# pxl-th/Trace.jl

Hardware: AMD Instinct MI355X
Metric: Mray/s (all bounces) (higher is better)
Workload: dtype f32

## Files before the change

### trace.jl_amd/csrc/th_kernels.h

```cpp
#pragma once
#include "th_device.h"

namespace th {

constexpr int kBlock = 256;
constexpr int kStackLds = 32;
constexpr int kStackSpill = 32;

struct PathQueue {
    float4* o;
    float4* d;
    float4* beta;
};
struct ShadowQueue {
    float4* o;
    float4* d;
    float4* c;
};
constexpr int kMaxDepth = 62;
constexpr int kSeg = 32;
constexpr uint32_t kSegGran = 256;
#ifndef TH_CTR_STRIDE
#define TH_CTR_STRIDE 32
#endif
// ... 111 lines not shown
#else
    return p;
#endif
}
TH_D size_t film_index(uint32_t layout, uint32_t npix, uint32_t spp, uint32_t s, uint32_t pix) {
    return layout ? ((size_t)(pix >> 6) * spp + s) * 64u + film_chunk_pos(pix & 63u) : (size_t)s * npix + pix;
}
struct MapSpp {
    const uint32_t* counts;
    uint32_t max_spp;
};
TH_D uint32_t spp_of_frame(uint32_t spp) { return spp; }
TH_D uint32_t spp_of_frame(const MapSpp& m) { return m.max_spp; }
TH_D uint32_t spp_of_pixel(uint32_t spp, uint32_t) { return spp; }
TH_D uint32_t spp_of_pixel(const MapSpp& m, uint32_t pix) { return m.counts[pix]; }
constexpr uint32_t kFilmPackSide = 0x80000000u;
constexpr uint32_t kFilmPackOverflow = 0xffffffffu;
constexpr uint32_t kFilmPackException = 0xffffffffu;
struct FilmSideTable {
    uint4* desc;
    uint32_t* count;
    uint32_t cap;
};
TH_D uint32_t film_pack_word(const FilmSideTable& side, uint4 d, int px, int py);
TH_D uint4 film_splat_desc(const DeviceSensor& se, int px, int py, uint64_t key) {
    const float rx = se.filter_radius[0], ry = se.filter_radius[1];
    const float inv_rx = 1.0f / rx, inv_ry = 1.0f / ry;
    const float pfx = (float)px + ts_uniform(key, TS_DIM_FILM_X), pfy = (float)py + ts_uniform(key, TS_DIM_FILM_Y);
    const float dpx = pfx - 0.5f, dpy = pfy - 0.5f;
    const float p0x = __builtin_ceilf(dpx - rx), p0y = __builtin_ceilf(dpy - ry);
    const float p1x = __builtin_floorf(dpx + rx) + 1.0f, p1y = __builtin_floorf(dpy + ry) + 1.0f;
    const int nx = (int)(p1x - p0x) + 1, ny = (int)(p1y - p0y) + 1;
    uint32_t oxw = 0, oyw = 0;
    for (int c = 0; c < 8; ++c) {
        const float X = p0x + (float)c, Y = p0y + (float)c;
        oxw |= (uint32_t)((int)jclamp(__builtin_ceilf(fabs_((X - dpx) * inv_rx * 16.0f)), 1.0f, 16.0f) - 1) << (4 * c);
        oyw |= (uint32_t)((int)jclamp(__builtin_floorf(fabs_((Y - dpy) * inv_ry * 16.0f)), 1.0f, 16.0f) - 1) << (4 * c);
    }
    return make_uint4(((uint32_t)(int)p0x & 0xffffu) | ((uint32_t)(int)p0y << 16), (uint32_t)nx | ((uint32_t)ny << 8), oxw, oyw);
}
TH_D uint32_t film_pack_desc(uint4 d, int px, int py) {
    const int p0x = (int)(short)(d.x & 0xffffu), p0y = (int)(short)(d.x >> 16);
    const uint32_t nx = d.y & 0xffu, ny = (d.y >> 8) & 0xffu;
    const int ox = px - p0x, oy = py - p0y;
    if (ox < 0 || ox > 1 || oy < 0 || oy > 1 || nx < 1u || nx > 3u || ny < 1u || ny > 3u) return kFilmPackException;
    return (uint32_t)ox | ((uint32_t)oy << 1) | ((nx - 1u) << 2) | ((ny - 1u) << 4) | ((d.z & 0xfffu) << 6) | ((d.w & 0xfffu) << 18);
}
TH_D uint32_t film_pack_word(const FilmSideTable& side, uint4 d, int px, int py) {
    const uint32_t w = film_pack_desc(d, px, py);
    if (w != kFilmPackException) return w;
    const uint32_t j = atomicAdd(side.count, 1u);
    if (j >= side.cap || j >= 0x7fffffffu) return kFilmPackOverflow;
    side.desc[j] = d;
    return kFilmPackSide | j;
}

TH_D void generate_ray(const DeviceSensor& se, f2 film, f2 lens, float time_u, f3& o, f3& d, float& time) {
    const f3 p_camera = xf_point(se.raster_to_camera, mk3(film.x, film.y, 0.0f));
    o = splat3(0.0f);
    d = normalize(p_camera);
    if (se.lens_radius > 0.0f) {
        const f2 pl = concentric_sample_disk(lens);
        const f2 p_lens{se.lens_radius * pl.x, se.lens_radius * pl.y};
        const float t = se.focal_distance / d.z;
        const f3 p_focus = o + d * t;
        o = mk3(p_lens.x, p_lens.y, 0.0f);
        d = normalize(p_focus - o);
    }
    time = (1 - time_u) * se.shutter_open + time_u * se.shutter_close;
    o = xf_point(se.camera_to_world, o);
    d = xf_vec(se.camera_to_world, d);
    d = normalize(d);
}

struct MapJobs {
    const uint32_t* jobs;
    uint32_t job0;
};
TH_D uint32_t raygen_slot(uint32_t slot0, uint32_t i) { return slot0 + i; }
TH_D uint32_t raygen_slot(const MapJobs& m, uint32_t i) { return m.jobs[m.job0 + i]; }
template <int TH_ONE_COPY = 0, class SLOT0 = uint32_t> __global__ __launch_bounds__(kBlock) void k_raygen(const DeviceSensor* __restrict__ sep, SLOT0 slot0, uint32_t n, uint64_t seed, uint32_t sample_offset,
                                                   PathQueue q, uint32_t cap, Counters* ctr, float4* __restrict__ Lf = nullptr, uint32_t spp_frame = 0, FilmSideTable side = FilmSideTable{nullptr, nullptr, 0}) {
    const DeviceSensor& se = *sep;
    for (uint32_t i = blockIdx.x * kBlock + threadIdx.x; i < n; i += gridDim.x * kBlock) {
        uint32_t slot = raygen_slot(slot0, i);
        const SlotInfo si = slot_info(se, slot);
        const uint64_t key = ts_stream_key(seed, si.px, si.py, sample_offset + si.sample);
        if (Lf) {
            slot = (uint32_t)film_index(1u, (uint32_t)(se.sb_w * se.band_rows), spp_frame, si.sample, si.pix);
            Lf[slot] = make_float4(0.0f, 0.0f, 0.0f, __uint_as_float(film_pack_word(side, film_splat_desc(se, si.px, si.py, key), si.px, si.py)));
        }
        const f2 film{(float)si.px + ts_uniform(key, TS_DIM_FILM_X), (float)si.py + ts_uniform(key, TS_DIM_FILM_Y)};
        const f2 lens{ts_uniform(key, TS_DIM_LENS_X), ts_uniform(key, TS_DIM_LENS_Y)};
        f3 o, d;
        float time;
        generate_ray(se, film, lens, ts_uniform(key, TS_DIM_TIME), o, d, time);
        d = check_direction(d);
        const uint32_t w = i >> 6;
        const uint32_t phys = (w % kSeg) * cap + (w / kSeg) * 64u + (i & 63u);
        q.o[phys] = make_float4(o.x, o.y, o.z, __uint_as_float(slot));
        q.d[phys] = make_float4(d.x, d.y, d.z, __uint_as_float((uint32_t)key));
        q.beta[phys] = make_float4(1.0f, 1.0f, 1.0f, __uint_as_float((uint32_t)(key >> 32)));
    }
    if (blockIdx.x == 0 && threadIdx.x < kSeg) {
        const uint32_t sgm = threadIdx.x, W = (n + 63u) >> 6;
        uint32_t cnt = ((W + kSeg - 1 - sgm) / kSeg) * 64u;
        if (W > 0 && (W - 1) % kSeg == sgm && (n & 63u)) cnt -= 64u - (n & 63u);
        ctr->n_queue[0][sgm * kCtrStride] = cnt;
    }
}

template <int TH_ONE_COPY = 0> __global__ __launch_bounds__(kBlock) void k_apply_poison(float4* __restrict__ L, const uint8_t* __restrict__ poison, uint64_t n) {
    for (uint64_t i = (uint64_t)blockIdx.x * kBlock + threadIdx.x; i < n; i += (uint64_t)gridDim.x * kBlock) {
        const uint32_t p = poison[i];
        if (p) {
            float4 l = L[i];
            const float nanv = __builtin_nanf("");
            if (p & 1u) l.x += nanv;
            if (p & 2u) l.y += nanv;
            if (p & 4u) l.z += nanv;
            L[i] = l;
        }
    }
}

struct Hit {
    float t;
    int prim;
    float b1, b2;
};
TH_D bool slab_test(float4 n0, float4 n1, f3 o, f3 inv_d, bool negx, bool negy, bool negz, float t_max) {
    float tx_min = ((negx ? n1.x : n0.x) - o.x) * inv_d.x;
    float tx_max = ((negx ? n0.x : n1.x) - o.x) * inv_d.x;
    const float ty_min = ((negy ? n1.y : n0.y) - o.y) * inv_d.y;
    const float ty_max = ((negy ? n0.y : n1.y) - o.y) * inv_d.y;
    if (tx_min > ty_max || ty_min > tx_max) return false;
    if (ty_min > tx_min) tx_min = ty_min;
    if (ty_max > tx_max) tx_max = ty_max;
    const float tz_min = ((negz ? n1.z : n0.z) - o.z) * inv_d.z;
    const float tz_max = ((negz ? n0.z : n1.z) - o.z) * inv_d.z;
    if (tx_min > tz_max || tz_min > tx_max) return false;
    if (tz_min > tx_min) tx_min = tz_min;
    if (tz_max < tx_max) tx_max = tz_max;
    return tx_min < t_max && tx_max > 0.0f;
}

template <bool ANY, bool COUNT>
TH_D bool traverse(const DeviceScene& sc, f3 o, f3 d, float t_max, uint32_t (*stk)[kBlock], Hit* hit, uint32_t& n_nodes, uint32_t& n_prims) {
    const f3 inv_d = mk3(1.0f / d.x, 1.0f / d.y, 1.0f / d.z);
    const bool negx = d.x < 0.0f, negy = d.y < 0.0f, negz = d.z < 0.0f;
    uint32_t spill[kStackSpill];
    int sp = 0;
    uint32_t cur = 0;
    bool found = false;
    if (sc.n_nodes == 0) return false;
    const uint32_t tid = threadIdx.x;
    while (true) {
        const float4 n0 = sc.nodes[2 * cur], n1 = sc.nodes[2 * cur + 1];
        if (COUNT) n_nodes++;
        bool pop = true;
        if (slab_test(n0, n1, o, inv_d, negx, negy, negz, t_max)) {
            const uint32_t a = __float_as_uint(n0.w), flags = __float_as_uint(n1.w);
            if ((flags & 3u) == 3u) {
                const uint32_t cnt = flags >> 2;
                for (uint32_t k = 0; k < cnt; ++k) {
                    const uint32_t slot = a + k;
                    const float4 p0 = sc.prims[3 * slot];
                    const uint32_t meta = __float_as_uint(p0.w);
                    if (COUNT) n_prims++;
                    if (meta & PRIM_SPHERE) {
                        SphereHit sh;
                        if (sphere_intersect<false>(sc.spheres[__float_as_uint(p0.x)], o, d, t_max, sh)) {
                            if (ANY) return true;
                            t_max = sh.t;
                            found = true;
                            hit->prim = (int)slot;
                            hit->b1 = hit->b2 = 0.0f;
                        }
                    } else {
                        const float4 p1 = sc.prims[3 * slot + 1], p2 = sc.prims[3 * slot + 2];
                        TriTest tt;
                        if (tri_intersect<!ANY>(mk3(p0.x, p0.y, p0.z), mk3(p1.x, p1.y, p1.z), mk3(p2.x, p2.y, p2.z), o, d, t_max, &tt)) {
                            if (ANY) return true;
                            t_max = tt.t;
                            found = true;
                            hit->prim = (int)slot;
                            hit->b1 = tt.bary.x;
                            hit->b2 = tt.bary.y;
                        }
                    }
                }
            } else {
                const uint32_t axis = flags & 3u;
                const bool neg = axis == 0 ? negx : (axis == 1 ? negy : negz);
                const uint32_t far_child = neg ? cur + 1 : a;
                cur = neg ? a : cur + 1;
                if (sp < kStackLds)
                    stk[sp][tid] = far_child;
                else if (sp < kStackLds + kStackSpill)
                    spill[sp - kStackLds] = far_child;
                sp++;
                pop = false;
            }
        }
        if (pop) {
            if (sp == 0) break;
            sp--;
            cur = sp < kStackLds ? stk[sp][tid] : (sp < kStackLds + kStackSpill ? spill[sp - kStackLds] : 0u);
        }
    }
    if (!ANY) hit->t = t_max;
    return found;
}

template <bool COUNT>
__global__ __launch_bounds__(kBlock) void k_trace_closest(DeviceScene sc, SegQueue q, const float4* __restrict__ ro, const float4* __restrict__ rd, const float* __restrict__ tmax_or_null,
                                                          float4* __restrict__ hits, Counters* ctr) {
    __shared__ uint32_t stk[kStackLds][kBlock];
    __shared__ SegView sv;
    seg_load(q, sv);
    const uint32_t total = sv.prefix[kSeg];
    uint32_t nn = 0, np = 0;
    uint32_t seg = 0;
    for (uint32_t flat = blockIdx.x * kBlock + threadIdx.x; flat < total; flat += gridDim.x * kBlock) {
        uint32_t lb;
        seg_locate_from(sv, flat & ~63u, seg, lb);
        const uint32_t local = lb + (flat & 63u);
        if (local >= sv.count[seg]) continue;
        const uint32_t i = seg_phys(q, seg, local);
        const float4 o4 = ro[i], d4 = rd[i];
        Hit h;
        h.prim = -1;
        h.b1 = h.b2 = 0.0f;
        const float t0 = tmax_or_null ? tmax_or_null[i] : kInf;
        const bool found = traverse<false, COUNT>(sc, mk3(o4.x, o4.y, o4.z), mk3(d4.x, d4.y, d4.z), t0, stk, &h, nn, np);
        hits[i] = make_float4(found ? h.t : kInf, __int_as_float(found ? h.prim : -1), h.b1, h.b2);
    }
    if (ctr) {
        if (blockIdx.x == 0 && threadIdx.x == 0) atomicAdd(&ctr->closest_total, (unsigned long long)seg_total(sv));
        if (COUNT) {
            const unsigned long long sn = wave_sum(nn), spr = wave_sum(np);
            if (lane_id() == 0) {
                atomicAdd(&ctr->nodes_closest, sn);
                atomicAdd(&ctr->prims_closest, spr);
            }
        }
    }
}

template <bool COUNT>
__global__ __launch_bounds__(kBlock) void k_trace_any(DeviceScene sc, SegQueue q, const float4* __restrict__ ro, const float4* __restrict__ rd, const float4* __restrict__ contrib,
                                                      const float* __restrict__ tmax_or_null, float4* __restrict__ L, uint8_t* __restrict__ occluded, Counters* ctr) {
    __shared__ uint32_t stk[kStackLds][kBlock];
    __shared__ SegView sv;
    seg_load(q, sv);
    const uint32_t total = sv.prefix[kSeg];
    uint32_t nn = 0, np = 0;
    uint32_t seg = 0;
    for (uint32_t flat = blockIdx.x * kBlock + threadIdx.x; flat < total; flat += gridDim.x * kBlock) {
        uint32_t lb;
        seg_locate_from(sv, flat & ~63u, seg, lb);
        const uint32_t local = lb + (flat & 63u);
        if (local >= sv.count[seg]) continue;
        const uint32_t i = seg_phys(q, seg, local);
        const float4 o4 = ro[i], d4 = rd[i];
        const float t0 = tmax_or_null ? tmax_or_null[i] : kInf;
        const bool occ = traverse<true, COUNT>(sc, mk3(o4.x, o4.y, o4.z), mk3(d4.x, d4.y, d4.z), t0, stk, nullptr, nn, np);
        if (L) {
            const uint32_t slot = __float_as_uint(o4.w);
            if (!occ) {
                const float4 c = contrib[i];
                float4 l = L[slot];
                l.x += c.x;
                l.y += c.y;
                l.z += c.z;
                L[slot] = l;
            } else {
                const uint32_t poison = __float_as_uint(d4.w);
                if (poison) {
                    float4 l = L[slot];
                    const float nanv = __builtin_nanf("");
                    if (poison & 1u) l.x += nanv;
                    if (poison & 2u) l.y += nanv;
                    if (poison & 4u) l.z += nanv;
                    L[slot] = l;
                }
            }
        } else {
            occluded[i] = occ ? 1 : 0;
        }
    }
    if (ctr) {
        if (blockIdx.x == 0 && threadIdx.x == 0) atomicAdd(&ctr->shadow_total, (unsigned long long)seg_total(sv));
        if (COUNT) {
            const unsigned long long sn = wave_sum(nn), spr = wave_sum(np);
            if (lane_id() == 0) {
                atomicAdd(&ctr->nodes_shadow, sn);
                atomicAdd(&ctr->prims_shadow, spr);
            }
        }
    }
}

template <bool TRI_ONLY = false, bool TAN = true>
TH_D bool rebuild_shading(const DeviceScene& sc, int prim, f3 o, f3 d, Shading& sh, uint32_t& material, const float4* bary = nullptr, f3* fast_r = nullptr) {
    const float4* rec = sc.shade + 8 * (size_t)prim;
    const float4 p0 = rec[0], p1 = rec[1], p2 = rec[2];
    const float4 na = rec[3], nb = rec[4], nc = rec[5];
    const float4 cn = rec[6], cs = rec[7];
    const uint32_t meta = __float_as_uint(p0.w);
    material = meta & PRIM_MATERIAL_MASK;
    if (fast_r) *fast_r = mk3(na.w, nb.w, nc.w);
    if (!TRI_ONLY && (meta & PRIM_SPHERE)) {
        const SphereRec& s = sc.spheres[__float_as_uint(p0.x)];
        SphereHit h;
        if (!sphere_intersect<true>(s, o, d, kInf, h)) return false;
        sh = shade_sphere(s, h, d);
        return true;
    }
    const f3 v0 = mk3(p0.x, p0.y, p0.z), v1 = mk3(p1.x, p1.y, p1.z), v2 = mk3(p2.x, p2.y, p2.z);
    TriTest tt;
    if (bary)
        tt.bary = mk3(bary->z, bary->w, bary->x);
    else if (!tri_intersect<true>(v0, v1, v2, o, d, kInf, &tt))
        return false;
    const bool has_n = (meta & PRIM_HAS_NORMALS) != 0;
    const TriConstants tc{mk3(cn.x, cn.y, cn.z), mk3(cs.x, cs.y, cs.z)};
    const float4* tan = (TAN && sc.tri_tan && (meta & PRIM_HAS_TANGENTS)) ? sc.tri_tan + 3 * (size_t)prim : nullptr;
    sh = shade_triangle(v0, v1, v2, has_n, mk3(na.x, na.y, na.z), mk3(nb.x, nb.y, nb.z), mk3(nc.x, nc.y, nc.z), (meta & PRIM_FLIP) != 0, tt.bary, d, &tc, tan);
    return true;
}
template <int TH_ONE_COPY = 0> __global__ __launch_bounds__(kBlock) void k_shade_constants(float4* __restrict__ shade, const float4* __restrict__ prims, const float4* __restrict__ nrm, const float4* __restrict__ uv, uint32_t n_prims) {
    for (uint32_t k = blockIdx.x * kBlock + threadIdx.x; k < n_prims; k += gridDim.x * kBlock) {
        float4* rec = shade + 8 * (size_t)k;
        const float4 p0 = prims[3 * (size_t)k], p1 = prims[3 * (size_t)k + 1], p2 = prims[3 * (size_t)k + 2];
        rec[0] = p0;
        rec[1] = p1;
        rec[2] = p2;
        for (int j = 0; j < 3; ++j) rec[3 + j] = nrm[3 * (size_t)k + j];
        float4 c6 = make_float4(0.0f, 0.0f, 0.0f, 0.0f), c7 = c6;
        if (!(__float_as_uint(p0.w) & PRIM_SPHERE)) {
            float uvs[6];
            bool has_uv = false;
            if (uv) {
                const float4 a = uv[2 * (size_t)k], b = uv[2 * (size_t)k + 1];
                uvs[0] = a.x, uvs[1] = a.y, uvs[2] = a.z, uvs[3] = a.w, uvs[4] = b.x, uvs[5] = b.y;
                has_uv = b.z != 0.0f;
            }
            const TriConstants tc = triangle_constants(mk3(p0.x, p0.y, p0.z), mk3(p1.x, p1.y, p1.z), mk3(p2.x, p2.y, p2.z), has_uv ? uvs : nullptr);
            c6 = make_float4(tc.n.x, tc.n.y, tc.n.z, 0.0f);
            c7 = make_float4(tc.ss.x, tc.ss.y, tc.ss.z, 0.0f);
        }
        rec[6] = c6;
        rec[7] = c7;
    }
}

#ifndef TH_SHADE_WAVES
#define TH_SHADE_WAVES 4
#endif
struct ShadeStream {
    const uint32_t* tags_in;
    uint32_t* tags_out;
    uint32_t term_stride;
    uint8_t* poison;
};
struct ShadeOut {
    bool want_shadow, want_next;
    float4 so4, sd4, sc4, no4, nd4, nb4;
    uint32_t next_depth;
};
template <bool STREAM, bool FAST, bool TAN = true, bool DIRL = false>
TH_D void shade_vertex(const DeviceScene& sc, const PathQueue& qin, const float4* __restrict__ hits, float4* __restrict__ L, uint32_t i, int depth_fixed, int max_depth,
                       uint32_t hits_have_bary, const ShadeStream& ss, ShadeOut& out) {
    const float4 h4 = hits[i];
    const int prim = __float_as_int(h4.y);
    const float4 o4 = qin.o[i], d4 = qin.d[i], b4 = qin.beta[i];
    const int depth = STREAM ? (int)ss.tags_in[i] : depth_fixed;
    const uint32_t slot = STREAM ? (uint32_t)(depth - 1) * ss.term_stride + __float_as_uint(o4.w) : __float_as_uint(o4.w);
    const f3 o = mk3(o4.x, o4.y, o4.z), d = mk3(d4.x, d4.y, d4.z);
    f3 beta = mk3(b4.x, b4.y, b4.z);
    Shading sh;
    uint32_t material;
    f3 fast_r;
    if (!(rebuild_shading<FAST, TAN>(sc, prim, o, d, sh, material, hits_have_bary ? &h4 : nullptr, &fast_r) && material != PRIM_NO_MATERIAL)) return;
    const LobeSet& bsdf = sc.materials[FAST ? 0u : material].set[1];
    const bool lambert = FAST || bsdf_is_single_lambert(bsdf);
    Lobe lam;
    if (FAST) {
        lam.kind = LOBE_LAMBERT_R;
        lam.type = BSDF_DIFFUSE | BSDF_REFLECTION;
        lam.r[0] = fast_r.x;
        lam.r[1] = fast_r.y;
        lam.r[2] = fast_r.z;
    } else if (lambert) {
        lam = bsdf.lobe[0];
    }
    const uint64_t key = ((uint64_t)__float_as_uint(b4.w) << 32) | (uint64_t)__float_as_uint(d4.w);
    const uint32_t v = (uint32_t)(depth - 1);
    const f3 wo = -d;
    const uint32_t poison = ((isnan_(beta.x) || isinf_(beta.x)) ? 1u : 0u) | ((isnan_(beta.y) || isinf_(beta.y)) ? 2u : 0u) | ((isnan_(beta.z) || isinf_(beta.z)) ? 4u : 0u);
    bool direct_added = false;
    if (sc.n_lights > 0) {
        const int nl = (int)sc.n_lights;
        int ln = (int)__builtin_ceilf(ts_uniform(key, ts_vertex_dim(v, TS_V_LIGHT_PICK)) * (float)nl);
        if (ln > nl) ln = nl;
        if (ln < 1) ln = 1;
        const float light_pdf = 1.0f / (float)nl;
        const LightRec light = nl == 1 ? uniform_load(sc.lights, 0u) : sc.lights[ln - 1];
        const LightSample ls = sample_li<DIRL>(light, sh.p);
        if (ls.pdf > 0.0f && !is_black(ls.radiance)) {
            const f3 f = (lambert ? lambert_bsdf_f(lam, sh, sh.wo, ls.wi) : bsdf_f(bsdf, sh, sh.wo, ls.wi, BSDF_ALL & ~BSDF_SPECULAR)) * fabs_(dot(ls.wi, sh.ns));
            if (!is_black(f)) {
                const f3 fl = f * ls.radiance;
                const f3 Ld1 = splat3(0.0f) + (ls.pdf == 1.0f ? fl : fl / ls.pdf);
                const f3 Ld = light_pdf == 1.0f ? Ld1 : Ld1 / light_pdf;
                const f3 c = beta * Ld;
                const f3 lp = light_target<DIRL>(light, sh.p);
                const f3 dir = lp - sh.p;
                const f3 org = sh.p + 1e-6f * dir;
                const f3 cd = check_direction(dir);
                out.so4 = make_float4(org.x, org.y, org.z, __uint_as_float(slot));
                out.sd4 = make_float4(cd.x, cd.y, cd.z, __uint_as_float(poison));
                out.sc4 = make_float4(c.x, c.y, c.z, 0.0f);
                out.want_shadow = true;
                direct_added = true;
            }
        }
    }
    if (!direct_added && poison && ss.poison) {
        ss.poison[slot] |= (uint8_t)poison;
    } else if (!direct_added && poison) {
        float4 l = L[slot];
        const float nanv = __builtin_nanf("");
        if (poison & 1u) l.x += nanv;
        if (poison & 2u) l.y += nanv;
        if (poison & 4u) l.z += nanv;
        L[slot] = l;
    }
    if (depth < max_depth) {
        const f2 u{ts_uniform(key, ts_vertex_dim(v, TS_V_BSDF_U0)), ts_uniform(key, ts_vertex_dim(v, TS_V_BSDF_U1))};
        const BsdfSample bs = lambert ? lambert_bsdf_sample_f(lam, sh, wo, u) : bsdf_sample_f(bsdf, sh, wo, u, BSDF_ALL);
        if (!(bs.pdf == 0.0f || is_black(bs.f))) {
            beta = beta * (bs.f * fabs_(dot(bs.wi, sh.ns)) / bs.pdf);
            const float by = to_Y(beta);
            bool alive = true;
            if (by < 0.25f) {
                const float cont = jmin(1.0f, by);
                if (ts_uniform(key, ts_vertex_dim(v, TS_V_RR)) > cont)
                    alive = false;
                else
                    beta = beta / cont;
            }
            if (alive) {
                const f3 org = sh.p + 1e-6f * bs.wi;
                const f3 nd = check_direction(bs.wi);
                out.no4 = make_float4(org.x, org.y, org.z, o4.w);
                out.nd4 = make_float4(nd.x, nd.y, nd.z, d4.w);
                out.nb4 = make_float4(beta.x, beta.y, beta.z, b4.w);
                out.next_depth = (uint32_t)(depth + 1);
                out.want_next = true;
            }
        }
    }
}

template <bool STREAM, bool TAN = true, bool DIRL = false>
__global__ __launch_bounds__(kBlock) __attribute__((amdgpu_waves_per_eu(TH_SHADE_WAVES))) void k_shade_path(DeviceScene sc, const DeviceSensor* __restrict__ sep, PathQueue qin, PathQueue qout, ShadowQueue sq, uint32_t cap,
                                                       const float4* __restrict__ hits, float4* __restrict__ L, Counters* ctr, int row, int depth_fixed, int max_depth, uint32_t hits_have_bary,
                                                       ShadeStream ss) {
    __shared__ SegView sv;
    __shared__ uint32_t s_ring[kBlock / 64][128];
    const SegQueue qv{ctr->n_queue[row], cap, 0u};
    seg_load(qv, sv);
    const uint32_t total = sv.prefix[kSeg];
    const uint32_t lane = lane_id(), wv = threadIdx.x >> 6;
    const unsigned long long lt_mask = (1ull << lane) - 1ull;
    const uint32_t seg_out = ((blockIdx.x * kBlock + threadIdx.x) >> 6) % kSeg;
    uint32_t ring_head = 0, ring_cnt = 0;
    auto emit = [&](const ShadeOut& e) {
        uint32_t si, ni;
        wave_compact2(e.want_shadow, &ctr->n_shadow[row][seg_out * kCtrStride], e.want_next, &ctr->n_queue[row + 1][seg_out * kCtrStride], si, ni);
        si += seg_out * cap;
        ni += seg_out * cap;
        if (e.want_shadow) {
            sq.o[si] = e.so4;
            sq.d[si] = e.sd4;
            sq.c[si] = e.sc4;
        }
        if (e.want_next) {
            qout.o[ni] = e.no4;
            qout.d[ni] = e.nd4;
            qout.beta[ni] = e.nb4;
            if (STREAM) ss.tags_out[ni] = e.next_depth;
        }
    };
    uint32_t seg_in = 0;
    for (uint32_t flat = blockIdx.x * kBlock + threadIdx.x; flat < total; flat += gridDim.x * kBlock) {
        uint32_t lb;
        seg_locate_from(sv, flat & ~63u, seg_in, lb);
        const uint32_t local = lb + (flat & 63u);
        const uint32_t i = seg_in * cap + local;
        int cls = 0;
        if (local < sv.count[seg_in]) {
            const int prim = __float_as_int(hits[i].y);
            if (prim >= 0) {
                cls = (__float_as_uint(sc.shade[8 * (size_t)prim].w) & PRIM_FAST) ? 1 : 2;
            }
        }
        ShadeOut e;
        e.want_shadow = e.want_next = false;
        e.next_depth = 0;
        if (cls == 1) shade_vertex<STREAM, true, TAN, DIRL>(sc, qin, hits, L, i, depth_fixed, max_depth, hits_have_bary, ss, e);
        emit(e);
        const unsigned long long m2 = __ballot(cls == 2);
        if (m2) {
            if (cls == 2) s_ring[wv][(ring_head + ring_cnt + (uint32_t)__popcll(m2 & lt_mask)) & 127u] = i;
            ring_cnt += (uint32_t)__popcll(m2);
            __builtin_amdgcn_fence(__ATOMIC_ACQ_REL, "wavefront");
            if (ring_cnt >= 64u) {
                const uint32_t j = s_ring[wv][(ring_head + lane) & 127u];
                ShadeOut g;
                g.want_shadow = g.want_next = false;
                g.next_depth = 0;
                shade_vertex<STREAM, false, TAN, DIRL>(sc, qin, hits, L, j, depth_fixed, max_depth, hits_have_bary, ss, g);
                emit(g);
                ring_head = (ring_head + 64u) & 127u;
                ring_cnt -= 64u;
                __builtin_amdgcn_fence(__ATOMIC_ACQ_REL, "wavefront");
            }
        }
    }
    if (ring_cnt) {
        ShadeOut g;
        g.want_shadow = g.want_next = false;
        g.next_depth = 0;
        if (lane < ring_cnt) shade_vertex<STREAM, false, TAN, DIRL>(sc, qin, hits, L, s_ring[wv][(ring_head + lane) & 127u], depth_fixed, max_depth, hits_have_bary, ss, g);
        emit(g);
    }
}
template <int TH_ONE_COPY = 0> __global__ __launch_bounds__(kBlock) void k_fold_terms(const float4* __restrict__ terms, uint64_t n_slots, uint32_t n_depths, float4* __restrict__ L) {
    for (uint64_t i = (uint64_t)blockIdx.x * kBlock + threadIdx.x; i < n_slots; i += (uint64_t)gridDim.x * kBlock) {
        float4 l = make_float4(0.0f, 0.0f, 0.0f, 0.0f);
        for (uint32_t dd = 0; dd < n_depths; ++dd) {
            const float4 t = terms[(uint64_t)dd * n_slots + i];
            l.x += t.x;
            l.y += t.y;
            l.z += t.z;
        }
        L[i] = l;
    }
}
template <int TH_ONE_COPY = 0> __global__ __launch_bounds__(kBlock) void k_fill_u32(uint32_t* __restrict__ p, uint64_t n, uint32_t v) {
    for (uint64_t i = (uint64_t)blockIdx.x * kBlock + threadIdx.x; i < n; i += (uint64_t)gridDim.x * kBlock) p[i] = v;
}

template <int TH_ONE_COPY = 0> __global__ __launch_bounds__(kBlock) void k_film_transpose(const float4* __restrict__ L, uint32_t npix, uint32_t spp, float4* __restrict__ Lt) {
    const uint32_t groups = (npix + 63u) >> 6;
    const uint64_t chunks = (uint64_t)groups * spp;
    const uint32_t lane = threadIdx.x & 63u;
    for (uint64_t c = ((uint64_t)blockIdx.x * kBlock + threadIdx.x) >> 6; c < chunks; c += ((uint64_t)gridDim.x * kBlock) >> 6) {
        const uint32_t s = (uint32_t)(c / groups), g = (uint32_t)(c - (uint64_t)s * groups);
        const uint32_t pix = g * 64u + lane;
        if (pix < npix) Lt[film_index(1u, npix, spp, s, pix)] = L[(size_t)s * npix + pix];
    }
}
template <int TH_ONE_COPY = 0> __global__ __launch_bounds__(kBlock) void k_film_positions(const DeviceSensor* __restrict__ sep, uint64_t n, uint64_t seed, uint32_t sample_offset, float2* __restrict__ pfilm, uint32_t layout,
                                                           uint32_t spp) {
    const DeviceSensor& se = *sep;
    for (uint64_t slot = (uint64_t)blockIdx.x * kBlock + threadIdx.x; slot < n; slot += (uint64_t)gridDim.x * kBlock) {
        const SlotInfo si = slot_info(se, (uint32_t)slot);
        const uint64_t key = ts_stream_key(seed, si.px, si.py, sample_offset + si.sample);
        pfilm[film_index(layout, (uint32_t)(se.sb_w * se.band_rows), spp, si.sample, si.pix)] = make_float2((float)si.px + ts_uniform(key, TS_DIM_FILM_X), (float)si.py + ts_uniform(key, TS_DIM_FILM_Y));
    }
}
template <int TH_ONE_COPY = 0> __global__ __launch_bounds__(kBlock) void k_film_gather(const DeviceSensor* __restrict__ sep, const float* __restrict__ table, const float4* __restrict__ L,
                                                        const float2* __restrict__ pfilm, uint32_t spp, uint32_t layout, float4* __restrict__ out) {
    const DeviceSensor& se = *sep;
    const uint32_t npx = (uint32_t)(se.film_w * se.film_h);
    const uint32_t npix = (uint32_t)(se.sb_w * se.band_rows);
    const float rx = se.filter_radius[0], ry = se.filter_radius[1];
    const float inv_rx = 1.0f / rx, inv_ry = 1.0f / ry;
    for (uint32_t idx = blockIdx.x * kBlock + threadIdx.x; idx < npx; idx += gridDim.x * kBlock) {
        const int fy = (int)(idx / (uint32_t)se.film_w), fx = (int)(idx - (uint32_t)fy * (uint32_t)se.film_w);
        const float X = se.crop_min[0] + (float)fx, Y = se.crop_min[1] + (float)fy;
        int sx_lo = (int)__builtin_floorf(X - 1.5f - rx), sx_hi = (int)__builtin_ceilf(X + rx + 0.5f);
        int sy_lo = (int)__builtin_floorf(Y - 1.5f - ry), sy_hi = (int)__builtin_ceilf(Y + ry + 0.5f);
        sx_lo = max(sx_lo, se.sb_min[0]);
        sy_lo = max(sy_lo, se.sb_min[1]);
        sx_hi = min(sx_hi, se.sb_max[0]);
        sy_hi = min(sy_hi, se.sb_max[1]);
        f3 xyz = splat3(0.0f);
        float wsum = 0.0f;
        if (se.accumulate) {
            const float4 prev = out[idx];
            xyz = mk3(prev.x, prev.y, prev.z);
            wsum = prev.w;
        }
        if (sx_lo <= sx_hi && sy_lo <= sy_hi) {
            const int ty_lo = max((sy_lo - se.sb_min[1]) >> 4, se.band_ty0), ty_hi = min((sy_hi - se.sb_min[1]) >> 4, se.band_ty1);
            const int tx_lo = (sx_lo - se.sb_min[0]) >> 4, tx_hi = (sx_hi - se.sb_min[0]) >> 4;
            for (int ty = ty_lo; ty <= ty_hi; ++ty)
                for (int tx = tx_lo; tx <= tx_hi; ++tx) {
                    const float tbx0 = (float)se.sb_min[0] + (float)tx * 16.0f, tby0 = (float)se.sb_min[1] + (float)ty * 16.0f;
                    const float tbx1 = jmin(tbx0 + 15.0f, (float)se.sb_max[0]), tby1 = jmin(tby0 + 15.0f, (float)se.sb_max[1]);
                    const float bx0 = jmax(__builtin_ceilf(tbx0 - 0.5f - rx), se.crop_min[0]), by0 = jmax(__builtin_ceilf(tby0 - 0.5f - ry), se.crop_min[1]);
                    const float bx1 = jmin(__builtin_floorf(tbx1 - 0.5f + rx) + 1.0f, se.crop_max[0]), by1 = jmin(__builtin_floorf(tby1 - 0.5f + ry) + 1.0f, se.crop_max[1]);
                    if (X < bx0 || X > bx1 || Y < by0 || Y > by1) continue;
                    f3 csum = splat3(0.0f);
                    float fws = 0.0f;
                    const int y0 = max(sy_lo, (int)tby0), y1 = min(sy_hi, (int)tby1);
                    const int x0 = max(sx_lo, (int)tbx0), x1 = min(sx_hi, (int)tbx1);
                    for (int sy = y0; sy <= y1; ++sy)
                        for (int sx = x0; sx <= x1; ++sx) {
                            const uint32_t pix = (uint32_t)(sy - se.band_y0) * (uint32_t)se.sb_w + (uint32_t)(sx - se.sb_min[0]);
                            for (uint32_t s = 0; s < spp; ++s) {
                                const float2 pf = pfilm[film_index(layout, npix, spp, s, pix)];
                                const float dpx = pf.x - 0.5f, dpy = pf.y - 0.5f;
                                float p0x = __builtin_ceilf(dpx - rx), p0y = __builtin_ceilf(dpy - ry);
                                float p1x = __builtin_floorf(dpx + rx) + 1.0f, p1y = __builtin_floorf(dpy + ry) + 1.0f;
                                p0x = jmax(p0x, jmax(bx0, 1.0f));
                                p0y = jmax(p0y, jmax(by0, 1.0f));
                                p1x = jmin(p1x, bx1);
                                p1y = jmin(p1y, by1);
                                if (X < p0x || X > p1x || Y < p0y || Y > p1y) continue;
                                const float ffx = fabs_((X - dpx) * inv_rx * 16.0f), ffy = fabs_((Y - dpy) * inv_ry * 16.0f);
                                const int ox = (int)jclamp(__builtin_ceilf(ffx), 1.0f, 16.0f);
                                const int oy = (int)jclamp(__builtin_floorf(ffy), 1.0f, 16.0f);
                                const float w = table[(oy - 1) * 16 + (ox - 1)];
                                const float4 l4 = L[film_index(layout, npix, spp, s, pix)];
                                f3 l = mk3(l4.x, l4.y, l4.z);
                                if (has_nan(l)) l = splat3(0.0f);
                                csum = csum + l * 1.0f * w;
                                fws += w;
                            }
                        }
                    xyz = xyz + rgb_to_xyz(csum);
                    wsum += fws;
                }
        }
        out[idx] = make_float4(xyz.x, xyz.y, xyz.z, wsum);
    }
}

TH_D void film_tile_bounds(const DeviceSensor& se, int ty, int tx, float rx, float ry, float& bx0, float& by0, float& bx1, float& by1) {
    const float tbx0 = (float)se.sb_min[0] + (float)tx * 16.0f, tby0 = (float)se.sb_min[1] + (float)ty * 16.0f;
    const float tbx1 = jmin(tbx0 + 15.0f, (float)se.sb_max[0]), tby1 = jmin(tby0 + 15.0f, (float)se.sb_max[1]);
    bx0 = jmax(__builtin_ceilf(tbx0 - 0.5f - rx), se.crop_min[0]);
    by0 = jmax(__builtin_ceilf(tby0 - 0.5f - ry), se.crop_min[1]);
    bx1 = jmin(__builtin_floorf(tbx1 - 0.5f + rx) + 1.0f, se.crop_max[0]);
    by1 = jmin(__builtin_floorf(tby1 - 0.5f + ry) + 1.0f, se.crop_max[1]);
}

template <int BX, int BY, class SPP = uint32_t>
__global__ __launch_bounds__(kBlock) void k_film_gather_block(const DeviceSensor* __restrict__ sep, const float* __restrict__ table, const float4* __restrict__ L,
                                                              const float2* __restrict__ pfilm, SPP spp_arg, uint32_t layout, float4* __restrict__ out) {
    const DeviceSensor& se = *sep;
    const uint32_t spp_frame = spp_of_frame(spp_arg);
    __shared__ float s_table[256];
    for (uint32_t t = threadIdx.x; t < 256u; t += kBlock) s_table[t] = table[t];
    __syncthreads();
    const uint32_t npix = (uint32_t)(se.sb_w * se.band_rows);
    const float rx = se.filter_radius[0], ry = se.filter_radius[1];
    const float inv_rx = 1.0f / rx, inv_ry = 1.0f / ry;
    const uint32_t nbx = ((uint32_t)se.film_w + BX - 1) / BX, nby = ((uint32_t)se.film_h + BY - 1) / BY;
    for (uint32_t bidx = blockIdx.x * kBlock + threadIdx.x; bidx < nbx * nby; bidx += gridDim.x * kBlock) {
        const int fy0 = (int)(bidx / nbx) * BY, fx0 = (int)(bidx - (bidx / nbx) * nbx) * BX;
        float X[BX], Y[BY];
        for (int i = 0; i < BX; ++i) X[i] = se.crop_min[0] + (float)(fx0 + i);
        for (int j = 0; j < BY; ++j) Y[j] = se.crop_min[1] + (float)(fy0 + j);
        int sx_lo = max((int)__builtin_floorf(X[0] - 1.5f - rx), se.sb_min[0]), sx_hi = min((int)__builtin_ceilf(X[BX - 1] + rx + 0.5f), se.sb_max[0]);
        int sy_lo = max((int)__builtin_floorf(Y[0] - 1.5f - ry), se.sb_min[1]), sy_hi = min((int)__builtin_ceilf(Y[BY - 1] + ry + 0.5f), se.sb_max[1]);
        f3 xyz[BY][BX];
        float wsum[BY][BX];
        for (int j = 0; j < BY; ++j)
            for (int i = 0; i < BX; ++i) {
                xyz[j][i] = splat3(0.0f);
                wsum[j][i] = 0.0f;
                if (se.accumulate && fx0 + i < se.film_w && fy0 + j < se.film_h) {
                    const float4 prev = out[(size_t)(fy0 + j) * (size_t)se.film_w + (size_t)(fx0 + i)];
                    xyz[j][i] = mk3(prev.x, prev.y, prev.z);
                    wsum[j][i] = prev.w;
                }
            }
        if (sx_lo <= sx_hi && sy_lo <= sy_hi) {
            const int ty_lo = max((sy_lo - se.sb_min[1]) >> 4, se.band_ty0), ty_hi = min((sy_hi - se.sb_min[1]) >> 4, se.band_ty1);
            const int tx_lo = (sx_lo - se.sb_min[0]) >> 4, tx_hi = (sx_hi - se.sb_min[0]) >> 4;
            for (int ty = ty_lo; ty <= ty_hi; ++ty)
                for (int tx = tx_lo; tx <= tx_hi; ++tx) {
                    float bx0, by0, bx1, by1;
                    film_tile_bounds(se, ty, tx, rx, ry, bx0, by0, bx1, by1);
                    const float tbx0 = (float)se.sb_min[0] + (float)tx * 16.0f, tby0 = (float)se.sb_min[1] + (float)ty * 16.0f;
                    const float tbx1 = jmin(tbx0 + 15.0f, (float)se.sb_max[0]), tby1 = jmin(tby0 + 15.0f, (float)se.sb_max[1]);
                    bool in_tile[BY][BX];
                    bool any_in = false;
                    for (int j = 0; j < BY; ++j)
                        for (int i = 0; i < BX; ++i) {
                            in_tile[j][i] = !(X[i] < bx0 || X[i] > bx1 || Y[j] < by0 || Y[j] > by1);
                            any_in = any_in || in_tile[j][i];
                        }
                    if (!any_in) continue;
                    f3 csum[BY][BX];
                    float fws[BY][BX];
                    for (int j = 0; j < BY; ++j)
                        for (int i = 0; i < BX; ++i) {
                            csum[j][i] = splat3(0.0f);
                            fws[j][i] = 0.0f;
                        }
                    const int y0 = max(sy_lo, (int)tby0), y1 = min(sy_hi, (int)tby1);
                    const int x0 = max(sx_lo, (int)tbx0), x1 = min(sx_hi, (int)tbx1);
                    for (int sy = y0; sy <= y1; ++sy)
                        for (int sx = x0; sx <= x1; ++sx) {
                            const uint32_t pix = (uint32_t)(sy - se.band_y0) * (uint32_t)se.sb_w + (uint32_t)(sx - se.sb_min[0]);
                            const uint32_t spp = spp_of_pixel(spp_arg, pix);
                            auto splat = [&](float2 pf, float4 l4) {
                                const float dpx = pf.x - 0.5f, dpy = pf.y - 0.5f;
                                float p0x = __builtin_ceilf(dpx - rx), p0y = __builtin_ceilf(dpy - ry);
                                float p1x = __builtin_floorf(dpx + rx) + 1.0f, p1y = __builtin_floorf(dpy + ry) + 1.0f;
                                p0x = jmax(p0x, jmax(bx0, 1.0f));
                                p0y = jmax(p0y, jmax(by0, 1.0f));
                                p1x = jmin(p1x, bx1);
                                p1y = jmin(p1y, by1);
                                bool okx[BX], oky[BY];
                                bool anyx = false, anyy = false;
                                for (int i = 0; i < BX; ++i) {
                                    okx[i] = !(X[i] < p0x || X[i] > p1x);
                                    anyx = anyx || okx[i];
                                }
                                for (int j = 0; j < BY; ++j) {
                                    oky[j] = !(Y[j] < p0y || Y[j] > p1y);
                                    anyy = anyy || oky[j];
                                }
                                if (!(anyx && anyy)) return;
                                f3 l = mk3(l4.x, l4.y, l4.z);
                                if (has_nan(l)) l = splat3(0.0f);
                                int ox[BX], oy[BY];
                                for (int i = 0; i < BX; ++i) ox[i] = (int)jclamp(__builtin_ceilf(fabs_((X[i] - dpx) * inv_rx * 16.0f)), 1.0f, 16.0f) - 1;
                                for (int j = 0; j < BY; ++j) oy[j] = ((int)jclamp(__builtin_floorf(fabs_((Y[j] - dpy) * inv_ry * 16.0f)), 1.0f, 16.0f) - 1) * 16;
                                for (int j = 0; j < BY; ++j)
                                    for (int i = 0; i < BX; ++i)
                                        if (okx[i] && oky[j]) {
                                            const float w = s_table[oy[j] + ox[i]];
                                            csum[j][i] = csum[j][i] + l * 1.0f * w;
                                            fws[j][i] += w;
                                        }
                            };
#ifndef TH_FILM_UNROLL
#define TH_FILM_UNROLL 4
#endif
                            constexpr uint32_t kFilmUnroll = TH_FILM_UNROLL;
                            uint32_t s = 0;
                            for (; s + kFilmUnroll <= spp; s += kFilmUnroll) {
                                float2 pfv[kFilmUnroll];
                                float4 lv[kFilmUnroll];
#pragma unroll
                                for (uint32_t u = 0; u < kFilmUnroll; ++u) {
                                    const size_t at = film_index(layout, npix, spp_frame, s + u, pix);
                                    pfv[u] = pfilm[at];
                                    lv[u] = L[at];
                                }
#pragma unroll
                                for (uint32_t u = 0; u < kFilmUnroll; ++u) splat(pfv[u], lv[u]);
                            }
                            for (; s < spp; ++s) splat(pfilm[film_index(layout, npix, spp_frame, s, pix)], L[film_index(layout, npix, spp_frame, s, pix)]);
                        }
                    for (int j = 0; j < BY; ++j)
                        for (int i = 0; i < BX; ++i)
                            if (in_tile[j][i]) {
                                xyz[j][i] = xyz[j][i] + rgb_to_xyz(csum[j][i]);
                                wsum[j][i] += fws[j][i];
                            }
                }
        }
        for (int j = 0; j < BY; ++j)
            for (int i = 0; i < BX; ++i)
                if (fx0 + i < se.film_w && fy0 + j < se.film_h) out[(size_t)(fy0 + j) * (size_t)se.film_w + (size_t)(fx0 + i)] = make_float4(xyz[j][i].x, xyz[j][i].y, xyz[j][i].z, wsum[j][i]);
    }
}
template <int TH_ONE_COPY = 0> __global__ __launch_bounds__(kBlock) void k_film_positions_map(const DeviceSensor* __restrict__ sep, const uint32_t* __restrict__ jobs, uint64_t n, uint64_t seed,
                                                               uint32_t sample_offset, float2* __restrict__ pfilm) {
    const DeviceSensor& se = *sep;
    for (uint64_t i = (uint64_t)blockIdx.x * kBlock + threadIdx.x; i < n; i += (uint64_t)gridDim.x * kBlock) {
        const uint32_t slot = jobs[i];
        const SlotInfo si = slot_info(se, slot);
        const uint64_t key = ts_stream_key(seed, si.px, si.py, sample_offset + si.sample);
        pfilm[slot] = make_float2((float)si.px + ts_uniform(key, TS_DIM_FILM_X), (float)si.py + ts_uniform(key, TS_DIM_FILM_Y));
    }
}

struct SplatDesc {
    uint32_t origin;
    uint32_t count;
    uint32_t ox;
    uint32_t oy;
};
template <int TH_ONE_COPY = 0> __global__ __launch_bounds__(kBlock) void k_film_descriptors(const DeviceSensor* __restrict__ sep, uint64_t n, uint64_t seed, uint32_t sample_offset, uint4* __restrict__ desc) {
    const DeviceSensor& se = *sep;
    const float rx = se.filter_radius[0], ry = se.filter_radius[1];
    const float inv_rx = 1.0f / rx, inv_ry = 1.0f / ry;
    for (uint64_t slot = (uint64_t)blockIdx.x * kBlock + threadIdx.x; slot < n; slot += (uint64_t)gridDim.x * kBlock) {
        const SlotInfo si = slot_info(se, (uint32_t)slot);
        const uint64_t key = ts_stream_key(seed, si.px, si.py, sample_offset + si.sample);
        const float pfx = (float)si.px + ts_uniform(key, TS_DIM_FILM_X), pfy = (float)si.py + ts_uniform(key, TS_DIM_FILM_Y);
        const float dpx = pfx - 0.5f, dpy = pfy - 0.5f;
        const float p0x = __builtin_ceilf(dpx - rx), p0y = __builtin_ceilf(dpy - ry);
        const float p1x = __builtin_floorf(dpx + rx) + 1.0f, p1y = __builtin_floorf(dpy + ry) + 1.0f;
        const int nx = (int)(p1x - p0x) + 1, ny = (int)(p1y - p0y) + 1;
        uint32_t oxw = 0, oyw = 0;
        for (int c = 0; c < 8; ++c) {
            const float X = p0x + (float)c, Y = p0y + (float)c;
            oxw |= (uint32_t)((int)jclamp(__builtin_ceilf(fabs_((X - dpx) * inv_rx * 16.0f)), 1.0f, 16.0f) - 1) << (4 * c);
            oyw |= (uint32_t)((int)jclamp(__builtin_floorf(fabs_((Y - dpy) * inv_ry * 16.0f)), 1.0f, 16.0f) - 1) << (4 * c);
        }
        desc[slot] = make_uint4(((uint32_t)(int)p0x & 0xffffu) | ((uint32_t)(int)p0y << 16), (uint32_t)nx | ((uint32_t)ny << 8), oxw, oyw);
    }
}
template <int BY>
// ... 573 lines not shown
```

Before: 6045.

## Prefetch shade records and hit prims into LDS with async global_load_lds pipeline

Restructures the path-shading loop so each wave prefetches the next iteration's hit primitive indices and the 128-byte shading records into LDS with asynchronous global_load_lds, double-buffered two iterations ahead. The shading code then reads the record from LDS through a new rebuild_shading_rec variant instead of issuing dependent global loads. The intent is to hide the latency of the gather from hit to prim to shade record behind the current iteration's shading work. In exchange it uses more LDS per block (guarded by a static_assert to keep four blocks per CU), adds manual waitcnt handling, and relies on wave-uniform bases via readfirstlane.

```diff
diff --git a/trace.jl_amd/csrc/th_kernels.h b/trace.jl_amd/csrc/th_kernels.h
--- a/trace.jl_amd/csrc/th_kernels.h
+++ b/trace.jl_amd/csrc/th_kernels.h
@@ -437,12 +437,12 @@
     }
 }
 
+struct ShadeRec {
+    float4 p0, p1, p2, na, nb, nc, cn, cs;
+};
 template <bool TRI_ONLY = false, bool TAN = true>
-TH_D bool rebuild_shading(const DeviceScene& sc, int prim, f3 o, f3 d, Shading& sh, uint32_t& material, const float4* bary = nullptr, f3* fast_r = nullptr) {
-    const float4* rec = sc.shade + 8 * (size_t)prim;
-    const float4 p0 = rec[0], p1 = rec[1], p2 = rec[2];
-    const float4 na = rec[3], nb = rec[4], nc = rec[5];
-    const float4 cn = rec[6], cs = rec[7];
+TH_D bool rebuild_shading_rec(const DeviceScene& sc, int prim, const ShadeRec& r, f3 o, f3 d, Shading& sh, uint32_t& material, const float4* bary = nullptr, f3* fast_r = nullptr) {
+    const float4 p0 = r.p0, p1 = r.p1, p2 = r.p2, na = r.na, nb = r.nb, nc = r.nc, cn = r.cn, cs = r.cs;
     const uint32_t meta = __float_as_uint(p0.w);
     material = meta & PRIM_MATERIAL_MASK;
     if (fast_r) *fast_r = mk3(na.w, nb.w, nc.w);
@@ -464,6 +464,12 @@
     const float4* tan = (TAN && sc.tri_tan && (meta & PRIM_HAS_TANGENTS)) ? sc.tri_tan + 3 * (size_t)prim : nullptr;
     sh = shade_triangle(v0, v1, v2, has_n, mk3(na.x, na.y, na.z), mk3(nb.x, nb.y, nb.z), mk3(nc.x, nc.y, nc.z), (meta & PRIM_FLIP) != 0, tt.bary, d, &tc, tan);
     return true;
+}
+template <bool TRI_ONLY = false, bool TAN = true>
+TH_D bool rebuild_shading(const DeviceScene& sc, int prim, f3 o, f3 d, Shading& sh, uint32_t& material, const float4* bary = nullptr, f3* fast_r = nullptr) {
+    const float4* rec = sc.shade + 8 * (size_t)prim;
+    const ShadeRec r{rec[0], rec[1], rec[2], rec[3], rec[4], rec[5], rec[6], rec[7]};
+    return rebuild_shading_rec<TRI_ONLY, TAN>(sc, prim, r, o, d, sh, material, bary, fast_r);
 }
 template <int TH_ONE_COPY = 0> __global__ __launch_bounds__(kBlock) void k_shade_constants(float4* __restrict__ shade, const float4* __restrict__ prims, const float4* __restrict__ nrm, const float4* __restrict__ uv, uint32_t n_prims) {
     for (uint32_t k = blockIdx.x * kBlock + threadIdx.x; k < n_prims; k += gridDim.x * kBlock) {
@@ -494,6 +500,9 @@
 #ifndef TH_SHADE_WAVES
 #define TH_SHADE_WAVES 4
 #endif
+#ifndef TH_SHADE_STAGE
+#define TH_SHADE_STAGE 1
+#endif
 struct ShadeStream {
     const uint32_t* tags_in;
     uint32_t* tags_out;
@@ -505,20 +514,38 @@
     float4 so4, sd4, sc4, no4, nd4, nb4;
     uint32_t next_depth;
 };
-template <bool STREAM, bool FAST, bool TAN = true, bool DIRL = false>
+struct ShadeStaged {
+    float4 h4, o4, d4, b4;
+    uint32_t tag;
+    ShadeRec rec;
+};
+template <bool STREAM, bool FAST, bool TAN = true, bool DIRL = false, bool STAGED = false>
 TH_D void shade_vertex(const DeviceScene& sc, const PathQueue& qin, const float4* __restrict__ hits, float4* __restrict__ L, uint32_t i, int depth_fixed, int max_depth,
-                       uint32_t hits_have_bary, const ShadeStream& ss, ShadeOut& out) {
-    const float4 h4 = hits[i];
+                       uint32_t hits_have_bary, const ShadeStream& ss, ShadeOut& out, const ShadeStaged& st = ShadeStaged()) {
+    float4 h4, o4, d4, b4;
+    uint32_t tag = 0;
+    if constexpr (STAGED) {
+        h4 = st.h4, o4 = st.o4, d4 = st.d4, b4 = st.b4;
+        tag = st.tag;
+    } else {
+        h4 = hits[i];
+        o4 = qin.o[i], d4 = qin.d[i], b4 = qin.beta[i];
+        if (STREAM) tag = ss.tags_in[i];
+    }
     const int prim = __float_as_int(h4.y);
-    const float4 o4 = qin.o[i], d4 = qin.d[i], b4 = qin.beta[i];
-    const int depth = STREAM ? (int)ss.tags_in[i] : depth_fixed;
+    const int depth = STREAM ? (int)tag : depth_fixed;
     const uint32_t slot = STREAM ? (uint32_t)(depth - 1) * ss.term_stride + __float_as_uint(o4.w) : __float_as_uint(o4.w);
     const f3 o = mk3(o4.x, o4.y, o4.z), d = mk3(d4.x, d4.y, d4.z);
     f3 beta = mk3(b4.x, b4.y, b4.z);
     Shading sh;
     uint32_t material;
     f3 fast_r;
-    if (!(rebuild_shading<FAST, TAN>(sc, prim, o, d, sh, material, hits_have_bary ? &h4 : nullptr, &fast_r) && material != PRIM_NO_MATERIAL)) return;
+    bool rebuilt;
+    if constexpr (STAGED)
+        rebuilt = rebuild_shading_rec<FAST, TAN>(sc, prim, st.rec, o, d, sh, material, hits_have_bary ? &h4 : nullptr, &fast_r);
+    else
+        rebuilt = rebuild_shading<FAST, TAN>(sc, prim, o, d, sh, material, hits_have_bary ? &h4 : nullptr, &fast_r);
+    if (!(rebuilt && material != PRIM_NO_MATERIAL)) return;
     const LobeSet& bsdf = sc.materials[FAST ? 0u : material].set[1];
     const bool lambert = FAST || bsdf_is_single_lambert(bsdf);
     Lobe lam;
@@ -631,6 +658,82 @@
         }
     };
     uint32_t seg_in = 0;
+#if TH_SHADE_STAGE
+    __shared__ uint32_t s_prim[kBlock / 64][2][64];
+    __shared__ float4 s_rec[kBlock / 64][8][64];
+    static_assert(sizeof(SegView) + sizeof(s_ring) + sizeof(s_prim) + sizeof(s_rec) <= 38400, "k_shade_path's shared arrays no longer fit four blocks per CU (LDS comes in units of 1 280 bytes)");
+    const uint32_t wvu = (uint32_t)__builtin_amdgcn_readfirstlane((int)wv);
+    typedef const __attribute__((address_space(1))) void* gptr_t;
+    typedef __attribute__((address_space(3))) void* lptr_t;
+    struct Pos {
+        uint32_t base, rem;
+    };
+    auto locate = [&](uint32_t flat_wave) {
+        uint32_t lb;
+        seg_locate_from(sv, flat_wave, seg_in, lb);
+        seg_in = (uint32_t)__builtin_amdgcn_readfirstlane((int)seg_in);
+        const uint32_t n = sv.count[seg_in];
+        return Pos{(uint32_t)__builtin_amdgcn_readfirstlane((int)(seg_in * cap + lb)), (uint32_t)__builtin_amdgcn_readfirstlane((int)(n > lb ? n - lb : 0u))};
+    };
+    auto stage_prim = [&](uint32_t parity, const Pos& p) {
+        if (lane < p.rem) __builtin_amdgcn_global_load_lds((gptr_t)&hits[p.base + lane].y, (lptr_t)&s_prim[wvu][parity][0], 4, 0, 0);
+    };
+    auto stage_rec = [&](bool on, int prim) {
+        if (on) {
+            const gptr_t src = (gptr_t)(sc.shade + 8 * (size_t)prim);
+            char* const img = (char*)&s_rec[wvu][0][0];
+#define TH_STAGE_QUARTER(j) __builtin_amdgcn_global_load_lds(src, (lptr_t)(img + 1008 * (j)), 16, 16 * (j), 0)
+            TH_STAGE_QUARTER(0), TH_STAGE_QUARTER(1), TH_STAGE_QUARTER(2), TH_STAGE_QUARTER(3), TH_STAGE_QUARTER(4), TH_STAGE_QUARTER(5), TH_STAGE_QUARTER(6), TH_STAGE_QUARTER(7);
+#undef TH_STAGE_QUARTER
+        }
+    };
+    const uint32_t stride = gridDim.x * kBlock, end = (uint32_t)__builtin_amdgcn_readfirstlane((int)total);
+    uint32_t flat = (uint32_t)__builtin_amdgcn_readfirstlane((int)((blockIdx.x * kBlock + threadIdx.x) & ~63u));
+    Pos p0{0u, 0u}, p1{0u, 0u};
+    if (flat < end) {
+        p0 = locate(flat);
+        stage_prim(0u, p0);
+        if (flat + stride < end) {
+            p1 = locate(flat + stride);
+            stage_prim(1u, p1);
+        }
+        asm volatile("s_waitcnt vmcnt(0)" ::: "memory");
+        const int prim = lane < p0.rem ? (int)s_prim[wv][0][lane] : -1;
+        asm volatile("s_waitcnt lgkmcnt(0)" ::: "memory");
+        stage_rec(prim >= 0, prim);
+    }
+    for (uint32_t k = 0; flat < end; flat += stride, ++k) {
+        const uint32_t i = p0.base + lane;
+        asm volatile("s_waitcnt vmcnt(0)" ::: "memory");
+        ShadeStaged st;
+        st.rec.p0 = s_rec[wv][0][lane], st.rec.p1 = s_rec[wv][1][lane], st.rec.p2 = s_rec[wv][2][lane];
+        st.rec.na = s_rec[wv][3][lane], st.rec.nb = s_rec[wv][4][lane], st.rec.nc = s_rec[wv][5][lane];
+        st.rec.cn = s_rec[wv][6][lane], st.rec.cs = s_rec[wv][7][lane];
+        const int word = (int)s_prim[wv][k & 1u][lane], word1 = (int)s_prim[wv][(k & 1u) ^ 1u][lane];
+        const int prim = lane < p0.rem ? word : -1;
+        const bool more1 = flat + stride < end, more2 = more1 && flat + 2u * stride < end;
+        const int prim1 = lane < p1.rem ? word1 : -1;
+        int cls = 0;
+        if (prim >= 0) cls = (__float_as_uint(st.rec.p0.w) & PRIM_FAST) ? 1 : 2;
+        const uint32_t il = cls == 1 ? i : 0u;
+        st.h4 = hits[il];
+        st.o4 = qin.o[il];
+        st.d4 = qin.d[il];
+        st.b4 = qin.beta[il];
+        st.tag = STREAM ? ss.tags_in[il] : 0u;
+        Pos p2{0u, 0u};
+        if (more2) p2 = locate(flat + 2u * stride);
+        asm volatile("s_waitcnt lgkmcnt(0)" ::: "memory");
+        stage_rec(prim1 >= 0, prim1);
+        if (more2) stage_prim(k & 1u, p2);
+        p0 = p1;
+        p1 = p2;
+        ShadeOut e;
+        e.want_shadow = e.want_next = false;
+        e.next_depth = 0;
+        if (cls == 1) shade_vertex<STREAM, true, TAN, DIRL, true>(sc, qin, hits, L, i, depth_fixed, max_depth, hits_have_bary, ss, e, st);
+        emit(e);
+#else
     for (uint32_t flat = blockIdx.x * kBlock + threadIdx.x; flat < total; flat += gridDim.x * kBlock) {
         uint32_t lb;
         seg_locate_from(sv, flat & ~63u, seg_in, lb);
@@ -648,6 +751,7 @@
         e.next_depth = 0;
         if (cls == 1) shade_vertex<STREAM, true, TAN, DIRL>(sc, qin, hits, L, i, depth_fixed, max_depth, hits_have_bary, ss, e);
         emit(e);
+#endif
         const unsigned long long m2 = __ballot(cls == 2);
         if (m2) {
             if (cls == 2) s_ring[wv][(ring_head + ring_cnt + (uint32_t)__popcll(m2 & lt_mask)) & 127u] = i;
```

After: 6091 (median of 6 runs). About the same (+0.8%).
